# gavrissh/training-operator

Measured on AMD Instinct MI355X. Metric: job×node fit evals/sec + gang placements/sec, 1M-node inventory, 1/2/4/8 GPUs, higher is better.
Workload: dtype int64

## Files before the change

training-operator_amd/csrc/pe_ctx.h:

```cpp
#pragma once

#include <hip/hip_runtime.h>
#include <rccl/rccl.h>

#include <immintrin.h>
#include <pthread.h>
#include <sched.h>

#include <algorithm>
#include <atomic>
#include <cstdlib>
#include <cstring>
#include <exception>
#include <functional>
#include <memory>
#include <mutex>
#include <new>
#include <stdexcept>
#include <string>
#include <thread>
#include <vector>

#include "pe_hostx.h"
#include "pe_kernels.h"
#include "pe_ledger_plan.h"
#include "pe_resolver.h"
#include "pe_slice_plan.h"
#include "placement.h"

namespace pe_engine {

using pe::ReqRec;

template <class T>
struct DevBuf {
  T* p = nullptr;
  size_t n = 0;
  hipError_t ensure(size_t count, unsigned flags = 0) {
    if (count <= n && p) return hipSuccess;
    if (p) (void)hipFree(p);
    p = nullptr;
    n = 0;
    const size_t bytes = std::max<size_t>(count, 1) * sizeof(T);
    hipError_t e = hipErrorOutOfMemory;
    if (flags) {
      e = hipExtMallocWithFlags((void**)&p, bytes, flags);
      if (e != hipSuccess) (void)hipGetLastError();
    }
    if (e != hipSuccess) e = hipMalloc((void**)&p, bytes);
    if (e == hipSuccess) n = count;
    return e;
  }
  void release() {
    if (p) (void)hipFree(p);
    p = nullptr;
    n = 0;
  }
};

template <class T>
struct HostBuf {
  T* p = nullptr;
  T* dev = nullptr;
  size_t n = 0;
  hipError_t ensure(size_t count, unsigned flags = hipHostMallocDefault) {
    if (count <= n && p) return hipSuccess;
    if (p) (void)hipHostFree(p);
    p = dev = nullptr;
    n = 0;
    hipError_t e = hipHostMalloc((void**)&p, std::max<size_t>(count, 1) * sizeof(T), flags);
    if (e == hipSuccess) std::memset((void*)p, 0, std::max<size_t>(count, 1) * sizeof(T));
    if (e == hipSuccess) e = hipHostGetDevicePointer((void**)&dev, p, 0);
    if (e == hipSuccess) n = count;
    return e;
  }
  void release() {
    if (p) (void)hipHostFree(p);
    p = dev = nullptr;
    n = 0;
  }
};
constexpr unsigned kZeroCopy = hipHostMallocCoherent | hipHostMallocMapped;

class SpinWorker {
 public:
  explicit SpinWorker(int device) : th_([this, device] {
    (void)hipSetDevice(device);
    loop();
  }) {}
  ~SpinWorker() {
    while (state_.load(std::memory_order_acquire) == 1) _mm_pause();
    state_.store(3, std::memory_order_release);
    th_.join();
  }
  void pin(const cpu_set_t& set) { (void)pthread_setaffinity_np(th_.native_handle(), sizeof(set), &set); }
  void post(std::function<void()> f) {
    task_ = std::move(f);
    err_ = nullptr;
    posted_ = true;
    state_.store(1, std::memory_order_release);
  }
  bool busy() const { return state_.load(std::memory_order_acquire) == 1; }
  bool failed() const { return state_.load(std::memory_order_acquire) == 2 && err_ != nullptr; }
  void wait() {
    if (!posted_) return;
    posted_ = false;
    for (int spin = 0; state_.load(std::memory_order_acquire) != 2; ++spin)
      if (spin < 4096) _mm_pause();
      else std::this_thread::yield();
    state_.store(0, std::memory_order_relaxed);
    if (err_) std::rethrow_exception(err_);
  }

 private:
  void loop() {
    int idle = 0;
    for (;;) {
      const int st = state_.load(std::memory_order_acquire);
      if (st == 3) return;
      if (st != 1) {
        if (++idle < 4096) _mm_pause();
        else std::this_thread::yield();
        continue;
      }
      idle = 0;
      try {
        task_();
      } catch (...) {
        err_ = std::current_exception();
      }
      state_.store(2, std::memory_order_release);
    }
  }
  std::atomic<int> state_{0};
  bool posted_ = false;
  std::function<void()> task_;
  std::exception_ptr err_;
  std::thread th_;
};

class SpinQueue {
 public:
  static constexpr unsigned kCap = 8;
  explicit SpinQueue(int device) : th_([this, device] {
    (void)hipSetDevice(device);
    loop();
  }) {}
  ~SpinQueue() {
    while (busy()) _mm_pause();
    stop_.store(true, std::memory_order_release);
    th_.join();
  }
  void pin(const cpu_set_t& set) { (void)pthread_setaffinity_np(th_.native_handle(), sizeof(set), &set); }
  void post(std::function<void()> f) {
    const unsigned t = tail_.load(std::memory_order_relaxed);
    while (t - head_.load(std::memory_order_acquire) >= kCap) _mm_pause();
    q_[t % kCap] = std::move(f);
    tail_.store(t + 1, std::memory_order_release);
  }
  bool busy() const { return head_.load(std::memory_order_acquire) != tail_.load(std::memory_order_acquire); }
  bool failed() const { return failed_.load(std::memory_order_acquire); }
  void wait() {
    for (int spin = 0; busy(); ++spin)
      if (spin < 4096) _mm_pause();
      else std::this_thread::yield();
    if (failed_.load(std::memory_order_acquire)) {
      failed_.store(false, std::memory_order_relaxed);
      std::exception_ptr e = err_;
      err_ = nullptr;
      if (e) std::rethrow_exception(e);
    }
  }

 private:
  void loop() {
    int idle = 0;
    for (;;) {
      const unsigned h = head_.load(std::memory_order_relaxed);
      if (h == tail_.load(std::memory_order_acquire)) {
        if (stop_.load(std::memory_order_acquire)) return;
        if (++idle < 4096) _mm_pause();
        else std::this_thread::yield();
        continue;
      }
      idle = 0;
      if (!failed_.load(std::memory_order_relaxed)) {
        try {
          q_[h % kCap]();
        } catch (...) {
          err_ = std::current_exception();
          failed_.store(true, std::memory_order_release);
        }
      }
      q_[h % kCap] = nullptr;
      head_.store(h + 1, std::memory_order_release);
    }
  }
  std::function<void()> q_[kCap];
  std::atomic<unsigned> head_{0}, tail_{0};
  std::atomic<bool> failed_{false}, stop_{false};
  std::exception_ptr err_;
  std::thread th_;
};


struct PeError {
  int code;
  std::string msg;
};

[[noreturn]] inline void raise(int code, const std::string& msg) { throw PeError{code, msg}; }

inline void hipchk(hipError_t e, const char* what) {
  if (e != hipSuccess) raise(PE_EHIP, std::string(what) + ": " + hipGetErrorString(e));
}

inline void ncclchk(ncclResult_t r, const char* what) {
  if (r != ncclSuccess) raise(PE_ERCCL, std::string(what) + ": " + ncclGetErrorString(r));
}

inline double rccl_timeout_s() {
  const char* e = std::getenv("PE_RCCL_TIMEOUT_S");
  const double s = e ? std::atof(e) : 60.0;
  return s > 0 ? s : 60.0;
}

inline int64_t round_up(int64_t x, int64_t m) { return (x + m - 1) / m * m; }

constexpr int kMaxMergers = 7;
constexpr int PATH_I64 = 1, PATH_I32 = 2, PATH_CODED = 4, PATH_NO_THERM = 8, PATH_PLANES = 16, PATH_PLANES_BLOCKS = 32,
              PATH_LDS = 64;
constexpr int PATHS_ALL = PATH_I64 | PATH_I32 | PATH_CODED | PATH_PLANES | PATH_LDS;

struct AggSeg {
  int64_t j0;
  int32_t nj, ng, nc;
  int64_t bytes;
// ... 111 lines not shown
  pe::SlicePlan sl_plan;
  HostBuf<uint8_t> dm_hin;
  DevBuf<uint8_t> dm_in;
  DevBuf<uint8_t> dm_out;
  HostBuf<uint8_t> dm_hout;
  DevBuf<int32_t> dm_log;
  DevBuf<int32_t> dm_dom;
  DevBuf<int64_t> dm_seg;
  DevBuf<uint32_t> dm_segw;
  HostBuf<int32_t> dm_hoff;
  hipEvent_t dm_ev = nullptr;
  HostBuf<uint8_t> dm_hlarge;
  DevBuf<uint8_t> dm_large;
  DevBuf<int64_t> dm_scratch;
  DevBuf<int32_t> pp_place;
  DevBuf<uint64_t> ff_state;
  HostBuf<uint32_t> ff_hopen;
  pe::LedgerPlan ld_plan;
  HostBuf<pe::LedgerRec> ld_hin;
  DevBuf<pe::LedgerRec> ld_in;
  DevBuf<ReqRec> g_groups;
  DevBuf<uint64_t> g_cand, g_bound;
  DevBuf<int32_t> g_cnt;
  DevBuf<uint8_t> g_out, g_gath;
  DevBuf<int64_t> g_upd;
  DevBuf<uint64_t> g_kn;
  DevBuf<uint32_t> g_lo;
  HostBuf<ReqRec> h_groups, h_groups2;
  HostBuf<ReqRec> h_groupsx[2];
  HostBuf<uint8_t> h_outx[2];
  HostBuf<int64_t> h_updx[2];
  uint32_t walk_gen = 0;
  int pin_cpu = -2;
  HostBuf<uint8_t> h_out, h_out2, h_own;
  HostBuf<uint8_t> h_merged;
  HostBuf<uint8_t> h_xg[4];
  std::vector<const uint64_t*> x_lists;
  std::vector<int32_t> x_ns, x_hd;
  HostBuf<int64_t> h_upd;
  bool walk = true;
  int64_t resort_nodes = 20480;
  int64_t w_est = 0;
  struct WalkSet {
    DevBuf<uint64_t> sk, rmin;
    DevBuf<int64_t> sr, rmax;
    DevBuf<uint32_t> sl, pos, ror, inovl, ovidx, ovlab;
    DevBuf<int64_t> ovres;
    DevBuf<uint64_t> ovkn;
    DevBuf<int32_t> ovl, ovln;
    void release() {
      sk.release(); rmin.release(); sr.release(); rmax.release(); sl.release(); pos.release(); ror.release();
      inovl.release(); ovidx.release(); ovlab.release(); ovres.release(); ovkn.release(); ovl.release(); ovln.release();
    }
  } ws[2];
  int w_cur = 0;
  bool w_pending = false;
  int64_t w_pend_est = 0;
  int64_t w_pend_windows = 0;
  hipStream_t w_s2 = nullptr;
  hipEvent_t w_ev_snap = nullptr, w_ev_done = nullptr;
  DevBuf<uint64_t> w_kin;
  DevBuf<uint32_t> w_slow;
  DevBuf<uint8_t> w_temp;
  DevBuf<uint32_t> w_flush;
  DevBuf<unsigned long long> w_stat;
  DevBuf<uint64_t> g_xstatus;
  pe_stats stats{};

  ~pe_ctx() {
    (void)hipSetDevice(device);
    if (comm_abort.joinable()) comm_abort.join();
    if (stream) (void)hipStreamSynchronize(stream);
    res0.release(); res.release(); labels.release(); island.release(); n_upd.release();
    fit_jobs.release(); fit_jobs32.release(); res32.release(); mask.release();
    code_vals.release(); code_needs.release(); code_jobs.release(); code_x.release(); counts.release(); h_counts.release();
    planes.release(); plane_jobs.release();
    lds_spec_d.release(); lds_vals.release(); lds_codes.release(); lds_ranks.release(); lds_aux.release(); lds_slots.release(); lds_rows.release();
    a_stage.release(); a_outh.release(); a_segoff.release(); a_flag.release(); a_ctr.release();
    for (hipEvent_t e : a_ev) (void)hipEventDestroy(e);
    if (a_h2d) (void)hipStreamSynchronize(a_h2d);
    for (hipEvent_t e : a_ev_h2d) (void)hipEventDestroy(e);
    if (a_h2d) (void)hipStreamDestroy(a_h2d);
    a_dstage.release();
    a_jgo.release(); a_mm.release(); a_rep.release(); a_gco.release(); a_mem.release();
    a_req.release(); a_out.release(); a_fl.release(); a_pres.release(); a_ovf.release();
    aw_stage.release(); aw_outh.release(); aw_dev.release();
    cp_hshapes.release(); cp_hout.release(); cp_shapes.release(); cp_part.release(); cp_out.release();
    lv_leaf.release(); lv_upper.release(); lv_hslots.release(); lv_hnodes.release();
    lv_hin.release(); lv_in.release(); lv_out.release(); lv_hout.release(); lv_split.release(); lv_hsplit.release();
    dm_hin.release(); dm_in.release(); dm_out.release(); dm_hout.release(); dm_log.release(); dm_dom.release();
    dm_seg.release(); dm_segw.release(); dm_hoff.release(); dm_hlarge.release(); dm_large.release(); dm_scratch.release();
    pp_place.release(); ff_state.release(); ff_hopen.release();
    ld_hin.release(); ld_in.release();
    if (dm_ev) (void)hipEventDestroy(dm_ev);
    for (hipEvent_t e : cp_ev)
      if (e) (void)hipEventDestroy(e);
    g_groups.release(); g_cand.release(); g_bound.release(); g_cnt.release(); g_out.release(); g_gath.release();
    g_upd.release(); g_kn.release(); g_lo.release(); h_groups.release(); h_groups2.release(); h_out.release(); h_out2.release(); h_own.release(); h_merged.release(); h_upd.release();
    for (auto& x : h_xg) x.release();
    for (int i = 0; i < 2; ++i) {
      h_groupsx[i].release();
      h_outx[i].release();
      h_updx[i].release();
    }
    if (w_s2) (void)hipStreamSynchronize(w_s2);
    for (auto& x : ws) x.release();
    w_kin.release(); w_slow.release(); w_temp.release(); w_stat.release(); w_flush.release(); g_xstatus.release();
    if (w_ev_snap) (void)hipEventDestroy(w_ev_snap);
    if (w_ev_done) (void)hipEventDestroy(w_ev_done);
    if (w_s2) (void)hipStreamDestroy(w_s2);
    if (comm) (void)ncclCommDestroy(comm);
    if (stream) (void)hipStreamDestroy(stream);
  }
};

namespace pe_engine {

inline void rccl_abort(pe_ctx* ctx) {
  if (!ctx->comm) return;
  ncclComm_t c = ctx->comm;
  ctx->comm = nullptr;
  ctx->comm_aborted = true;
  const int dev = ctx->device;
  ctx->comm_abort = std::thread([c, dev] {
    (void)hipSetDevice(dev);
    (void)ncclCommAbort(c);
  });
}

template <class F>
int guarded(pe_ctx* ctx, F&& body) {
  if (!ctx) return PE_EINVAL;
  std::lock_guard<std::mutex> lk(ctx->mu);
  ctx->err.clear();
  try {
    hipchk(hipSetDevice(ctx->device), "hipSetDevice");
    return body();
  } catch (const PeError& e) {
    ctx->err = e.msg;
    return e.code;
// ... 96 lines not shown
```

training-operator_amd/csrc/pe_engine_greedy.cpp:

```cpp
#include <chrono>
#include <cstdio>
#include <deque>
#include <utility>

#include "pe_ctx.h"
#include "pe_greedy_mode.h"
#include "pe_merge.h"

namespace {

using Clock = std::chrono::steady_clock;
double ms(Clock::duration d) { return std::chrono::duration<double, std::milli>(d).count(); }
double us(Clock::duration d) { return std::chrono::duration<double, std::micro>(d).count(); }
double ms_since(Clock::time_point t) { return ms(Clock::now() - t); }
double us_since(Clock::time_point t) { return us(Clock::now() - t); }

const pe::GreedyLimits kLimits{pe::WK_ROUND,   pe::MG_CAP,  pe::MG_THREADS,        pe::RM_MAX_WORLD,
                               pe::RM_MAX_LDS, kMaxMergers, &pe::cand_group_bytes, &pe::merge_ranked_lds};

uint32_t next_gen(pe_ctx* ctx) {
  if (++ctx->walk_gen == 0) ++ctx->walk_gen;
  return ctx->walk_gen;
}

// ... 107 lines not shown
  hipchk(pe::launch_walk_switch(s, ctx->res.p, ctx->stride, ctx->labels.p, ctx->Ns, ctx->w_slow.p, walk_index(ctx, nx)),
         "launch walk_switch");
  ctx->w_cur = nx;
  ctx->w_pending = false;
  ctx->w_est = ctx->w_pend_est;
  ctx->stats.resorts += 1;
}

template <class At>
bool read_rank_lists(int W, int K, At group_at, const uint64_t** lists, int32_t* ns, uint64_t* L) {
  bool bad = false;
  *L = pe::NO_KEY;
  for (int r = 0; r < W; ++r) {
    const uint8_t* g = group_at(r);
    pe::CandHdr h;
    std::memcpy(&h, g, sizeof(h));
    *L = std::min(*L, h.limit);
    lists[r] = reinterpret_cast<const uint64_t*>(g + sizeof(h));
    bad |= h.n < 0 || h.n > K;
    ns[r] = std::max(0, std::min(h.n, K));
  }
  return !bad;
}

struct GreedyBatch {
  int64_t n_jobs, G;
  const int32_t *job_group_off, *priority, *group_count;
  const int64_t* group_req;
  const uint32_t* group_need;
};

struct Pin {
  cpu_set_t old_set, l3;
  bool on = false;
  Pin(bool no_pin, int rank, int world, int& picked) {
    if (no_pin || pthread_getaffinity_np(pthread_self(), sizeof(old_set), &old_set) != 0) return;
    if (world > 1 && picked == -2) picked = pe::l3_pick(old_set, rank);
    const int cpu = world > 1 ? picked : sched_getcpu();
    if (!pe::l3_cpus(cpu, &l3)) return;
    CPU_AND(&l3, &l3, &old_set);
    on = CPU_COUNT(&l3) >= 3 && pthread_setaffinity_np(pthread_self(), sizeof(l3), &l3) == 0;
  }
  ~Pin() {
    if (on) (void)pthread_setaffinity_np(pthread_self(), sizeof(old_set), &old_set);
  }
};

struct StreamIdle {
  hipStream_t s;
  const SpinQueue* x = nullptr;
  static bool stream_busy(hipStream_t s) {
    const hipError_t e = hipStreamQuery(s);
    if (e == hipErrorNotReady) return true;
    hipchk(e, "walk window stream");
    return false;
  }
  static bool busy(void* u) {
    auto* t = static_cast<StreamIdle*>(u);
    if (t->x && t->x->failed()) const_cast<SpinQueue*>(t->x)->wait();
    return (t->x && t->x->busy()) || stream_busy(t->s);
  }
};

struct DumpClose {
  FILE*& f;
  ~DumpClose() {
    if (f) std::fclose(f);
  }
};

struct TraceOut {
  int& helper_cpu;
  const bool& on;
  std::vector<double>& a; std::vector<double>& b; std::vector<double>& c;
  std::vector<double>& d; std::vector<double>& e; std::vector<double>& f;
  ~TraceOut() {
    if (!on || a.empty()) return;
    auto pr = [](const char* n, std::vector<double>& v) {
      if (v.empty()) return;
      std::sort(v.begin(), v.end());
      double sum = 0;
      for (double x : v) sum += x;
      std::fprintf(stderr, "%s n %zu sum %.2f ms mean %.1f us p10 %.1f p50 %.1f p90 %.1f max %.1f\n", n, v.size(),
                   sum / 1e3, sum / v.size(), v[v.size() / 10], v[v.size() / 2], v[v.size() * 9 / 10], v.back());
    };
    pr("wait   ", a);
    pr("resolve", b);
    pr("post   ", c);
    pr("xspin  ", d);
    pr("xmerge ", e);
    pr("xblock ", f);
    auto sib = [](int cpu) {
      char path[128], buf[64] = {0};
      std::snprintf(path, sizeof path, "/sys/devices/system/cpu/cpu%d/topology/thread_siblings_list", cpu);
      FILE* f = std::fopen(path, "r");
      if (f) {
        if (!std::fgets(buf, sizeof buf, f)) buf[0] = 0;
        std::fclose(f);
      }
      buf[std::strcspn(buf, "\n")] = 0;
      return std::string(buf);
    };
    const int mc = sched_getcpu();
    std::fprintf(stderr, "cpus: main %d (siblings %s) helper %d (siblings %s)\n", mc, sib(mc).c_str(), helper_cpu,
                 helper_cpu >= 0 ? sib(helper_cpu).c_str() : "-");
  }
};

struct EventsFree {
  std::vector<std::pair<hipEvent_t, hipEvent_t>>& v;
  ~EventsFree() {
    for (auto& p : v) {
      (void)hipEventDestroy(p.first);
      (void)hipEventDestroy(p.second);
    }
  }
};

struct XWait {
  std::unique_ptr<SpinQueue>& w;
  ~XWait() {
    if (w) try {
        w->wait();
      } catch (...) {
      }
  }
};

struct Flight {
  std::vector<int32_t> groups;
  pe::Cursor end;
  int buf = 0;
  size_t ver = 0;
};

struct GreedyRun {
  pe_ctx* const ctx;
  const pe::GreedyKnobs kn;
  const pe::GreedyMode m;
  pe::Resolver& R;
  const uint32_t* const group_need;
  pe_host_exchange* const hx;
  const hipStream_t s;
  const size_t gb;
  const int Wmax, nwaves;
  int k_win;
  const bool async_resort, wev, wflush;
  const int64_t kResortEarly, kResortLate;
  decltype(&pe::launch_merge_shards) const merge_fn;
  HostBuf<uint8_t>* const h_blob[4];
  HostBuf<ReqRec>* const h_req[4];
  uint8_t* outbuf(int b) const { return h_blob[b]->p; }
  uint8_t* outbufdev(int b) const { return h_blob[b]->dev; }
  HostBuf<ReqRec>& hgroups(int b) const { return *h_req[m.signalled ? b : 0]; }

  FILE* dump = nullptr;
  DumpClose dump_close{dump};
  int64_t dump_left;
  std::vector<double> tr_wait, tr_res, tr_post, tr_xspin, tr_xmerge, tr_xblock;
  int helper_cpu = -1;
  TraceOut trace_out{helper_cpu, kn.trace, tr_wait, tr_res, tr_post, tr_xspin, tr_xmerge, tr_xblock};
  std::vector<std::pair<hipEvent_t, hipEvent_t>> walk_events;
  EventsFree events_free{walk_events};
  int64_t walk_launch_groups = 0;
  std::vector<pe::GroupCands> cands;
  int cb = 0;
  std::unique_ptr<SpinWorker> worker;
  const Pin& pin;
  const uint8_t* last_blob = nullptr;
  uint32_t buf_gen[4] = {0, 0, 0, 0};
  int buf_k[4];
  pe::WindowFeed feed;
  StreamIdle stream_idle;
  const double coll_tmo;
  double feed_spin_seen = 0;
  std::unique_ptr<SpinQueue> xworker;
  std::vector<std::unique_ptr<SpinWorker>> xmergers;
  XWait xwait_exit{xworker};
  std::deque<Flight> fl;
  std::vector<std::vector<pe::Update>> hist;
  size_t n_app = 0;
  int next_buf = 0, upd_slot = 0;
  bool posted = false;
  std::vector<pe::Update> seed, upd;
  std::vector<std::pair<const std::vector<pe::Update>*, int>> to_apply;
  std::vector<Flight*> to_scan;
  Clock::time_point t_setup, t_loop;

  GreedyRun(pe_ctx* c, const GreedyBatch& batch, const pe::GreedyKnobs& knobs, const pe::GreedyMode& mode,
            pe::Resolver& resolver, const Pin& pinned)
      : ctx(c), kn(knobs), m(mode), R(resolver), group_need(batch.group_need),
        hx(pe::hx_is(c->exchange) ? static_cast<pe_host_exchange*>(c->exchange_user) : nullptr), s(c->stream),
        gb(pe::cand_group_bytes(mode.K)), Wmax(c->window_groups),
        nwaves((int)std::max<int64_t>(1, (c->Ns + pe::SC_SPAN - 1) / pe::SC_SPAN)), k_win(mode.K0),
        async_resort(mode.walk && knobs.async_resort), wev(mode.walk && knobs.walk_events),
        wflush(mode.walk && knobs.walk_flush), kResortEarly(std::min<int64_t>(4096, c->resort_nodes / 4)),
        kResortLate(std::max<int64_t>(1, c->resort_nodes / 2)),
        merge_fn(mode.ranked ? &pe::launch_merge_ranked : &pe::launch_merge_shards),
        h_blob{&c->h_out, &c->h_out2, &c->h_outx[0], &c->h_outx[1]},
        h_req{&c->h_groups, &c->h_groups2, &c->h_groupsx[0], &c->h_groupsx[1]}, dump_left(knobs.dump_max),
        pin(pinned), buf_k{mode.K, mode.K, mode.K, mode.K}, stream_idle{c->stream},
        coll_tmo(!mode.use_exchange && c->comm ? rccl_timeout_s() : 0.0) {
    open_dump(batch);
    if (m.pipelined) {
      worker.reset(new SpinWorker(ctx->device));
      if (pin.on) worker->pin(pin.l3);
    }
    if (pin.on) R.pin_helper(pin.l3);
    feed.idle = &StreamIdle::busy;
    feed.idle_user = &stream_idle;
    feed.timeout_s = coll_tmo;
    feed.on_timeout = [](void* u) { rccl_abort(static_cast<pe_ctx*>(u)); };
    feed.timeout_user = ctx;
    if (m.split_x) {
      xworker.reset(new SpinQueue(ctx->device));
      if (pin.on) xworker->pin(pin.l3);
      stream_idle.x = xworker.get();
      if (m.zc_host) {
        for (int t = 1; t < m.T; ++t) {
          xmergers.emplace_back(new SpinWorker(ctx->device));
          if (pin.on) xmergers.back()->pin(pin.l3);
          xmergers.back()->post(&pe::merge_warm);
        }
        xworker->post(&pe::merge_warm);
      }
    }
  }

  void open_dump(const GreedyBatch& b) {
    if (!kn.dump_path) return;
    dump = std::fopen(kn.dump_path, "wb");
    if (!dump) return;
    const int64_t hdr[3] = {b.n_jobs, b.G, (int64_t)m.K};
    std::fwrite(hdr, 8, 3, dump);
    std::fwrite(b.job_group_off, 4, (size_t)b.n_jobs + 1, dump);
    std::fwrite(b.priority, 4, (size_t)b.n_jobs, dump);
    std::fwrite(b.group_count, 4, (size_t)b.G, dump);
    std::fwrite(b.group_req, 8, (size_t)b.G * pe::D, dump);
    std::fwrite(b.group_need, 4, (size_t)b.G, dump);
    std::fwrite(&ctx->n_total, 8, 1, dump);
    std::fwrite(ctx->m_nodes.data(), sizeof(pe::NodeState), ctx->m_nodes.size(), dump);
  }

  void sync_stream(const char* what) {
    if (coll_tmo <= 0) return hipchk(hipStreamSynchronize(s), what);
    const auto ts = Clock::now();
    for (unsigned spin = 1;; ++spin) {
      const hipError_t e = hipStreamQuery(s);
      if (e != hipErrorNotReady) return hipchk(e, what);
      if (spin > 64) std::this_thread::sleep_for(std::chrono::microseconds(20));
      if ((spin & 63) == 0 && std::chrono::duration<double>(Clock::now() - ts).count() > coll_tmo) {
        rccl_abort(ctx);
        throw pe::CollectiveTimeout(std::string(what) + ": the stream did not drain within " +
// ... 118 lines not shown
    for (int t = 1; t < T; ++t) {
      Times* x = &tt[t];
      xmergers[(size_t)t - 1]->wait();
      xmergers[(size_t)t - 1]->post([&timed_share, t, x] { timed_share(t, x); });
    }
    std::exception_ptr err;
    try {
      timed_share(0, &tt[0]);
    } catch (...) {
      err = std::current_exception();
    }
    for (int t = 1; t < T; ++t) try {
        xmergers[(size_t)t - 1]->wait();
      } catch (...) {
        if (!err) err = std::current_exception();
      }
    if (err) std::rethrow_exception(err);
    double busy = 0, spun = 0, merged = 0;
    for (int t = 0; t < T; ++t) {
      busy = std::max(busy, tt[t].busy);
      spun += tt[t].spun;
      merged += tt[t].merged;
    }
    if (trace) {
      tr_xspin.push_back(spun);
      tr_xmerge.push_back(merged);
    }
    const double all_ms = ms_since(t0);
    ctx->stats.xchg_merge_ms += busy;
    ctx->stats.xchg_wait_ms += std::max(0.0, all_ms - busy);
    pe::hx_zc_consumed(hx, *hw);
  }

  void exchange_window(int b, int Wg, uint32_t gen, bool own_direct, const SpinWorker* launcher,
                       const pe::HxWindow* hw = nullptr) {
    if (m.zc_host) return exchange_window_zc(b, Wg, gen, hw);
    const int K = m.K;
    const size_t bytes = (size_t)Wg * gb;
    if (own_direct && ctx->Ns > 0) {
      struct Idle {
        const SpinWorker* l;
        hipStream_t s;
        static bool busy(void* u) {
          auto* x = static_cast<Idle*>(u);
          return (x->l && x->l->busy()) || StreamIdle::stream_busy(x->s);
        }
      } idle{launcher, s};
      pe::WindowFeed own;
      std::vector<pe::GroupCands> own_cands;
      own.idle = &Idle::busy;
      own.idle_user = &idle;
      own.reset(ctx->h_own.p, Wg, K, gen, &own_cands);
      own.wait((size_t)Wg - 1);
    } else {
      hipchk(hipMemcpyAsync(ctx->h_own.p, ctx->g_out.p, bytes, hipMemcpyDeviceToHost, s), "D2H cands");
      hipchk(hipStreamSynchronize(s), "sync own cands");
    }
    const auto tx = Clock::now();
    if (ctx->exchange(ctx->exchange_user, ctx->h_own.p, m.dev_merge ? ctx->h_xg[b].p : outbuf(b), bytes) != 0)
      raise(PE_ERCCL, "exchange callback failed");
    ctx->stats.xchg_wait_ms += ms_since(tx);
    if (m.xhost_merge) {
      const auto tm = Clock::now();
      for (int w = 0; w < Wg; ++w) host_merge_group(ctx->h_xg[b].p, Wg, w, outbuf(b), gen);
      ctx->stats.xchg_merge_ms += ms_since(tm);
    } else if (m.dev_merge) {
      hipchk(merge_fn(s, ctx->h_xg[b].dev, ctx->world, Wg, K, outbufdev(b), gen, 0, nullptr, true),
             "launch merge_shards");
    }
  }

  void launch_lists(const HostBuf<ReqRec>& hg, int b, int Wg, int Kw, uint8_t* dst, uint32_t gen, const pe::HxWindow& hw) {
    const int K = m.K;
    if (m.walk) {
// ... 206 lines not shown
  }

  void restart() {
    fl.clear();
    hist.clear();
    n_app = 0;
    next_buf = 0;
    Flight* f = add_flight(R.cursor());
    if (!f) return;
    if (m.split_x && m.zc_host) {
      const uint32_t gen = next_gen(ctx);
      const pe::HxWindow hw = pe::hx_zc_next(hx);
      enqueue_window(f->groups, f->buf, gen, true, &hw);
      const int b = f->buf, wg = (int)f->groups.size();
      xworker->post([this, b, wg, gen, hw] { exchange_window(b, wg, gen, true, worker.get(), &hw); });
    } else {
      enqueue_window(f->groups, f->buf);
    }
  }

  void plan_post() {
    to_apply.clear();
    to_scan.clear();
    for (; n_app < hist.size(); ++n_app) {
      to_apply.emplace_back(&hist[n_app], upd_slot);
      upd_slot = (upd_slot + 1) % m.upd_slots;
    }
    while ((int)fl.size() < m.depth + 1)
      if (Flight* f = add_flight(fl.back().end)) to_scan.push_back(f);
      else break;
  }

  void post_scan() {
    worker->post([this, to_apply = to_apply, to_scan = to_scan] {
      const auto tp = Clock::now();
      if (kn.trace) helper_cpu = sched_getcpu();
      for (const auto& a : to_apply) enqueue_apply(*a.first, a.second);
      for (Flight* f : to_scan) enqueue_window(f->groups, f->buf);
      if (kn.trace) tr_post.push_back(us_since(tp));
    });
  }

  void post_split() {
    plan_post();
    struct XWin {
      int buf, wg;
      uint32_t gen;
      pe::HxWindow hw;
    };
    std::vector<XWin> xs;
    std::vector<std::pair<Flight*, XWin>> ws;
    for (Flight* f : to_scan) {
      const uint32_t gen = next_gen(ctx);
      xs.push_back(XWin{f->buf, (int)f->groups.size(), gen, m.zc_host ? pe::hx_zc_next(hx) : pe::HxWindow{}});
      ws.emplace_back(f, xs.back());
    }
    const auto txb = Clock::now();
    if (!m.zc_host) xworker->wait();
    if (kn.trace) tr_xblock.push_back(us_since(txb));
    worker->post([this, to_apply = to_apply, ws] {
      const auto tp = Clock::now();
      if (kn.trace) helper_cpu = sched_getcpu();
      for (const auto& a : to_apply) enqueue_apply(*a.first, a.second);
      for (const auto& w : ws)
        enqueue_window(w.first->groups, w.first->buf, w.second.gen, true, m.zc_host ? &w.second.hw : nullptr);
      if (kn.trace) tr_post.push_back(us_since(tp));
    });
// ... 35 lines not shown
        try {
          worker->wait();
        } catch (...) {
        }
        if (xworker) xworker->wait();
        throw;
      }
      worker->wait();
      const bool landed = consumed && R.cursor() == cur.end && fl.size() > 1;
      if (landed && !R.done()) {
        hist.push_back(std::move(upd));
        upd = {};
        fl.pop_front();
        if (m.early_post) {
          plan_post();
          post_scan();
          posted = true;
        }
        continue;
      }
      if (xworker) xworker->wait();
      sync_stream("sync speculative");
      for (; n_app < hist.size(); ++n_app) {
        enqueue_apply(hist[n_app], 0);
        sync_stream("sync apply");
      }
      enqueue_apply(upd, 0);
      if (R.done()) break;
      if (!consumed) k_win = m.K;
      restart();
    }
    t_loop = Clock::now();
    if (xworker) xworker->wait();
    sync_stream("sync greedy");
    walk_drop_pending(ctx);
  }

  void walk_stats() {
    if (!m.walk) return;
    unsigned long long wc[2] = {0, 0};
    hipchk(hipMemcpy(wc, ctx->w_stat.p, sizeof(wc), hipMemcpyDeviceToHost), "D2H walk counters");
    ctx->stats.walk_rounds += (int64_t)wc[0];
    ctx->stats.walk_overlay += (int64_t)wc[1];
    ctx->stats.walk_groups += walk_launch_groups;
    ctx->stats.walk_prepass += walk_launch_groups * ((ctx->Ns + pe::WK_ROUND - 1) / pe::WK_ROUND);
    for (auto& p : walk_events) {
      float t = 0.f;
      hipchk(hipEventElapsedTime(&t, p.first, p.second), "event elapsed");
      ctx->stats.walk_ms += t;
    }
  }
};

int64_t check_batch(GreedyBatch& b, const int32_t* out_pod_node, const int32_t* out_job_status) {
  need_ptr(b.job_group_off, "job_group_off");
  need_ptr(b.priority, "priority");
  need_ptr(out_job_status, "out_job_status");
  check_offsets(b.job_group_off, b.n_jobs, -1, "job_group_off");
  b.G = b.job_group_off[b.n_jobs];
  int64_t P = 0;
  if (b.G > 0) {
    need_ptr(b.group_count, "group_count");
    need_ptr(b.group_req, "group_req");
    check_req(b.group_req, b.G, "group_req");
    for (int64_t g = 0; g < b.G; ++g) {
      if (b.group_count[g] < 0) raise(PE_EINVAL, "negative group_count");
      P += b.group_count[g];
    }
  }
  if (P > 0) need_ptr(out_pod_node, "out_pod_node");
  return P;
}

void prep_device(pe_ctx* ctx) {
  hipchk(ctx->g_kn.ensure((size_t)std::max<int64_t>(ctx->stride, 1)), "alloc node keys");
  hipchk(ctx->g_lo.ensure((size_t)2 * std::max<int64_t>(ctx->stride, 1)), "alloc node lows");
  hipchk(pe::launch_prep_nodes(ctx->stream, ctx->res.p, ctx->stride, ctx->Ns, (uint64_t)ctx->begin, ctx->g_kn.p,
                               ctx->g_lo.p),
         "launch prep_nodes");
  hipchk(ctx->w_stat.ensure(2), "alloc walk counters");
  hipchk(hipMemsetAsync(ctx->w_stat.p, 0, 2 * sizeof(unsigned long long), ctx->stream), "memset walk counters");
  if (ctx->walk && ctx->Ns > 0) walk_resort(ctx);
}

pe::GreedyFacts greedy_facts(const pe_ctx* ctx) {
  pe::GreedyFacts f;
  f.world = ctx->world;
  f.rank = ctx->rank;
  f.has_comm = ctx->comm != nullptr;
  f.has_exchange = ctx->exchange != nullptr;
  f.hx = pe::hx_is(ctx->exchange);
  f.hx_slot_bytes = f.hx ? pe::hx_slot_bytes(static_cast<const pe_host_exchange*>(ctx->exchange_user)) : 0;
  f.ctx_walk = ctx->walk;
  f.has_nodes = ctx->Ns > 0;
  f.pipeline = ctx->pipeline;
  f.topk = ctx->topk;
  f.window_groups = ctx->window_groups;
  return f;
}

bool zc_agreed(pe_ctx* ctx, int K) {
  pe_host_exchange* const hx = static_cast<pe_host_exchange*>(ctx->exchange_user);
  if (ctx->zc_hx != hx) {
    const uint8_t ok = ctx->world <= pe::HX_ZC_MAX_WORLD && pe::hx_zc_register(hx) &&
                               (size_t)ctx->window_groups * pe::cand_group_bytes(K) <= pe::hx_slot_bytes(hx) ? 1 : 0;
    std::vector<uint8_t> all((size_t)ctx->world, 0);
    if (ctx->exchange(ctx->exchange_user, &ok, all.data(), 1) != 0) raise(PE_ERCCL, "exchange callback failed");
    ctx->zc_ok = std::all_of(all.begin(), all.end(), [](uint8_t v) { return v == 1; });
    ctx->zc_hx = hx;
  }
  return ctx->zc_ok;
}

// ... 28 lines not shown
      hipchk(ctx->h_xg[b].ensure((size_t)Wmax * gb * ctx->world, kZeroCopy), "alloc pinned gathered");
}

}

extern "C" {

int pe_place_greedy(pe_ctx* ctx, int64_t n_jobs, const int32_t* job_group_off, const int32_t* priority,
                    const int32_t* group_count, const int64_t* group_req, const uint32_t* group_need,
                    int32_t* out_pod_node, int32_t* out_job_status) {
  return guarded(ctx, [&]() -> int {
    const auto t0 = Clock::now();
    if (!ctx->loaded) raise(PE_ESTATE, "no inventory loaded");
    if (ctx->comm_aborted)
      raise(PE_ERCCL, "the RCCL communicator was aborted after a window's all-gather timed out; recreate the context");
    if (n_jobs < 0) raise(PE_EINVAL, "n_jobs < 0");
    if (n_jobs == 0) return PE_OK;
    GreedyBatch batch{n_jobs, 0, job_group_off, priority, group_count, group_req, group_need};
    const int64_t P = check_batch(batch, out_pod_node, out_job_status);
    std::vector<uint32_t> no_need;
    if (!batch.group_need) {
      no_need.assign((size_t)std::max<int64_t>(batch.G, 1), 0u);
      batch.group_need = group_need = no_need.data();
    }
    prep_device(ctx);
    const auto t_prep = Clock::now();
    if (ctx->resolver) ctx->resolver->reset(n_jobs, job_group_off, priority, group_count, group_req, group_need);
    else ctx->resolver.reset(new pe::Resolver(n_jobs, job_group_off, priority, group_count, group_req, group_need));
    pe::Resolver& R = *ctx->resolver;
    R.set_mirror(pe::Mirror{ctx->m_nodes.data(), ctx->n_total});
    const auto t_res = Clock::now();

    const pe::GreedyKnobs kn = pe::GreedyKnobs::from_env();
    const Pin pin(kn.no_pin, ctx->rank, ctx->world, ctx->pin_cpu);
    const pe::GreedyFacts facts = greedy_facts(ctx);
    const bool zc = pe::greedy_zc_wanted(facts, kn, kLimits) && zc_agreed(ctx, pe::greedy_mode_base(facts, kn, kLimits).K);
    const pe::GreedyMode m = pe::greedy_mode(facts, kn, kLimits, zc);
    size_buffers(ctx, kn, m);

    GreedyRun run(ctx, batch, kn, m, R, pin);
    run.run();
    run.walk_stats();
    if (P > 0) std::memcpy(out_pod_node, R.pod_node().data(), (size_t)P * 4);
    std::memcpy(out_job_status, R.job_status().data(), (size_t)n_jobs * 4);
    ctx->stats.rescans += R.rescans();
    ctx->stats.pods_placed += R.pods_placed();
    ctx->stats.jobs_placed += R.jobs_placed();
    ctx->stats.jobs_failed += R.jobs_failed();
    ctx->stats.last_greedy_ms = ms_since(t0);
    if (kn.trace)
      std::fprintf(stderr, "greedy phases (us): checks+prep %.0f resolver %.0f setup %.0f loop %.0f tail %.0f\n",
                   us(t_prep - t0), us(t_res - t_prep), us(run.t_setup - t_res), us(run.t_loop - run.t_setup),
                   us_since(run.t_loop));
    return PE_OK;
  });
}

}
```

training-operator_amd/csrc/pe_resolver.cpp:

```cpp
#include "pe_resolver.h"

#include <algorithm>
#include <chrono>
#include <stdexcept>
#include <string>
#include <cstring>
#include <numeric>
#include <utility>
#include <cstdio>
#include <cstdlib>

#include <immintrin.h>
#include <pthread.h>
#include <sched.h>
#ifdef PE_RES_PROF
#include <x86intrin.h>
#endif

namespace pe {
#ifdef PE_RES_PROF
struct ResProf { long cgroups = 0, cskip = 0, cdirty = 0; unsigned long long p1 = 0, p2 = 0, p3 = 0, la = 0, ka = 0, st = 0, seed = 0, keys = 0, skip = 0, place = 0, fin = 0, other = 0; long skips = 0, pods = 0, groups = 0, dirty = 0, scored = 0, sready = 0, slocal = 0, sfull = 0;
  ~ResProf() { std::fprintf(stderr, "keys split: lookahead %.1fM keys_all %.1fM seed top %.1fM | place split: choose+fetch %.1fM m %.1fM upsert..key %.1fM\n", la / 1e6, ka / 1e6, st / 1e6, p1 / 1e6, p2 / 1e6, p3 / 1e6); std::fprintf(stderr, "cycles seed %.1fM keys %.1fM skip %.1fM place %.1fM fin %.1fM | skips %ld pods %ld | per group: dirty %.0f scored %.1f\n", seed / 1e6, keys / 1e6, skip / 1e6, place / 1e6, fin / 1e6, skips, pods, (double)dirty / groups, (double)scored / groups); std::fprintf(stderr, "seed tops: helper %ld local %ld full %ld\n", sready, slocal, sfull); std::fprintf(stderr, "window conflicts: %ld of %ld groups depend on an earlier group of their window (%ld via a skipped list entry, %ld via a chosen changed node)\n", cgroups, groups, cskip, cdirty); } };
static ResProf rp;
#define RP_T() __rdtsc()
// ... 480 lines not shown
    while (h < gc.size() && seeds.contains((int64_t)(gc.keys[h] & 0xFFFFFFull))) ++h;
  top.head = h;
  seeds.keys_all(q, need, gc.limit, out, idx);
  int n = 0;
  bool trunc = false;
  for (int32_t i : idx) {
    const uint64_t k = out[(size_t)i];
    if (k >= gc.limit) continue;
    if (n == SeedTop::kTop) {
      trunc = true;
      if (k >= top.key[n - 1]) continue;
      --n;
    }
    int j = n++;
    for (; j > 0 && top.key[j - 1] > k; --j) top.key[j] = top.key[j - 1];
    top.key[j] = k;
  }
  top.n = n;
  top.truncated = trunc;
}

SeedScorer::~SeedScorer() {
  if (!th_) return;
  stop();
  state_.store(3, std::memory_order_seq_cst);
  {
    std::lock_guard<std::mutex> lk(park_mu_);
    park_cv_.notify_one();
  }
  th_->join();
}

void SeedScorer::pin(const cpu_set_t& set) {
  pin_set_ = set;
  have_pin_ = true;
  if (th_) (void)pthread_setaffinity_np(th_->native_handle(), sizeof(set), &set);
}

void SeedScorer::start(const DirtySet* seeds, const std::vector<int32_t>* groups,
                       const std::vector<GroupCands>* cands, const int64_t* scan_req, const uint32_t* need,
                       const WindowFeed* feed, const NodeState* mirror, int64_t mirror_n) {
  seeds_ = seeds;
  mirror_ = mirror;
  mirror_n_ = mirror ? mirror_n : 0;
  groups_ = groups;
  cands_ = cands;
  feed_ = feed;
  req_ = scan_req;
  need_ = need;
  if (cap_ < groups->size()) {
    cap_ = std::max<size_t>(groups->size(), 2 * cap_);
    slots_.reset(new TopSlot[cap_]);
    gen_ = 0;
  }
  if (++gen_ == 0) {
    for (size_t i = 0; i < cap_; ++i) slots_[i].gen.store(0, std::memory_order_relaxed);
    gen_ = 1;
  }
  main_wi_.store(0, std::memory_order_relaxed);
  if (!th_) {
    th_.reset(new std::thread([this] { loop(); }));
#ifndef PE_SEED_TEST_YIELD
    cpu_set_t set;
    if (have_pin_) (void)pthread_setaffinity_np(th_->native_handle(), sizeof(pin_set_), &pin_set_);
    else if (l3_cpus(sched_getcpu(), &set)) (void)pthread_setaffinity_np(th_->native_handle(), sizeof(set), &set);
#endif
// ... 547 lines not shown
```

Before: 46470 billion.

## Persist parked helper threads across greedy calls and cache CPU pinning

Replaces the per-call SpinWorker and SpinQueue helper threads with persistent ParkedWorker and ParkedQueue objects stored in the context. Between calls they sleep on a condition variable and are woken by a lease when a run starts. The L3 affinity set is cached, and pthread_setaffinity is skipped when it would not change anything. The walk-counter readback becomes an async copy into pinned memory before the final sync, replacing a separate blocking hipMemcpy. This removes thread creation, join and redundant syscalls on every greedy call, at the cost of wake latency and more lifecycle complexity.

```diff
diff --git a/training-operator_amd/csrc/pe_ctx.h b/training-operator_amd/csrc/pe_ctx.h
--- a/training-operator_amd/csrc/pe_ctx.h
+++ b/training-operator_amd/csrc/pe_ctx.h
@@ -24,6 +24,7 @@
 #include "pe_hostx.h"
 #include "pe_kernels.h"
 #include "pe_ledger_plan.h"
+#include "pe_parked_worker.h"
 #include "pe_resolver.h"
 #include "pe_slice_plan.h"
 #include "placement.h"
@@ -82,127 +83,9 @@
 };
 constexpr unsigned kZeroCopy = hipHostMallocCoherent | hipHostMallocMapped;
 
-class SpinWorker {
- public:
-  explicit SpinWorker(int device) : th_([this, device] {
-    (void)hipSetDevice(device);
-    loop();
-  }) {}
-  ~SpinWorker() {
-    while (state_.load(std::memory_order_acquire) == 1) _mm_pause();
-    state_.store(3, std::memory_order_release);
-    th_.join();
-  }
-  void pin(const cpu_set_t& set) { (void)pthread_setaffinity_np(th_.native_handle(), sizeof(set), &set); }
-  void post(std::function<void()> f) {
-    task_ = std::move(f);
-    err_ = nullptr;
-    posted_ = true;
-    state_.store(1, std::memory_order_release);
-  }
-  bool busy() const { return state_.load(std::memory_order_acquire) == 1; }
-  bool failed() const { return state_.load(std::memory_order_acquire) == 2 && err_ != nullptr; }
-  void wait() {
-    if (!posted_) return;
-    posted_ = false;
-    for (int spin = 0; state_.load(std::memory_order_acquire) != 2; ++spin)
-      if (spin < 4096) _mm_pause();
-      else std::this_thread::yield();
-    state_.store(0, std::memory_order_relaxed);
-    if (err_) std::rethrow_exception(err_);
-  }
-
- private:
-  void loop() {
-    int idle = 0;
-    for (;;) {
-      const int st = state_.load(std::memory_order_acquire);
-      if (st == 3) return;
-      if (st != 1) {
-        if (++idle < 4096) _mm_pause();
-        else std::this_thread::yield();
-        continue;
-      }
-      idle = 0;
-      try {
-        task_();
-      } catch (...) {
-        err_ = std::current_exception();
-      }
-      state_.store(2, std::memory_order_release);
-    }
-  }
-  std::atomic<int> state_{0};
-  bool posted_ = false;
-  std::function<void()> task_;
-  std::exception_ptr err_;
-  std::thread th_;
-};
-
-class SpinQueue {
- public:
-  static constexpr unsigned kCap = 8;
-  explicit SpinQueue(int device) : th_([this, device] {
-    (void)hipSetDevice(device);
-    loop();
-  }) {}
-  ~SpinQueue() {
-    while (busy()) _mm_pause();
-    stop_.store(true, std::memory_order_release);
-    th_.join();
-  }
-  void pin(const cpu_set_t& set) { (void)pthread_setaffinity_np(th_.native_handle(), sizeof(set), &set); }
-  void post(std::function<void()> f) {
-    const unsigned t = tail_.load(std::memory_order_relaxed);
-    while (t - head_.load(std::memory_order_acquire) >= kCap) _mm_pause();
-    q_[t % kCap] = std::move(f);
-    tail_.store(t + 1, std::memory_order_release);
-  }
-  bool busy() const { return head_.load(std::memory_order_acquire) != tail_.load(std::memory_order_acquire); }
-  bool failed() const { return failed_.load(std::memory_order_acquire); }
-  void wait() {
-    for (int spin = 0; busy(); ++spin)
-      if (spin < 4096) _mm_pause();
-      else std::this_thread::yield();
-    if (failed_.load(std::memory_order_acquire)) {
-      failed_.store(false, std::memory_order_relaxed);
-      std::exception_ptr e = err_;
-      err_ = nullptr;
-      if (e) std::rethrow_exception(e);
-    }
-  }
-
- private:
-  void loop() {
-    int idle = 0;
-    for (;;) {
-      const unsigned h = head_.load(std::memory_order_relaxed);
-      if (h == tail_.load(std::memory_order_acquire)) {
-        if (stop_.load(std::memory_order_acquire)) return;
-        if (++idle < 4096) _mm_pause();
-        else std::this_thread::yield();
-        continue;
-      }
-      idle = 0;
-      if (!failed_.load(std::memory_order_relaxed)) {
-        try {
-          q_[h % kCap]();
-        } catch (...) {
-          err_ = std::current_exception();
-          failed_.store(true, std::memory_order_release);
-        }
-      }
-      q_[h % kCap] = nullptr;
-      head_.store(h + 1, std::memory_order_release);
-    }
-  }
-  std::function<void()> q_[kCap];
-  std::atomic<unsigned> head_{0}, tail_{0};
-  std::atomic<bool> failed_{false}, stop_{false};
-  std::exception_ptr err_;
-  std::thread th_;
-};
-
+inline std::function<void()> helper_init(int device) {
+  return [device] { (void)hipSetDevice(device); };
+}
 
 struct PeError {
   int code;
@@ -380,6 +263,11 @@
   HostBuf<int64_t> h_updx[2];
   uint32_t walk_gen = 0;
   int pin_cpu = -2;
+  cpu_set_t pin_l3;
+  int pin_l3_cpu = -1;
+  std::unique_ptr<pe::ParkedWorker> g_worker;
+  std::unique_ptr<pe::ParkedQueue> g_xworker;
+  std::vector<std::unique_ptr<pe::ParkedWorker>> g_xmergers;
   HostBuf<uint8_t> h_out, h_out2, h_own;
   HostBuf<uint8_t> h_merged;
   HostBuf<uint8_t> h_xg[4];
@@ -412,12 +300,16 @@
   DevBuf<uint8_t> w_temp;
   DevBuf<uint32_t> w_flush;
   DevBuf<unsigned long long> w_stat;
+  HostBuf<unsigned long long> h_wstat;
   DevBuf<uint64_t> g_xstatus;
   pe_stats stats{};
 
   ~pe_ctx() {
     (void)hipSetDevice(device);
     if (comm_abort.joinable()) comm_abort.join();
+    g_xmergers.clear();
+    g_xworker.reset();
+    g_worker.reset();
     if (stream) (void)hipStreamSynchronize(stream);
     res0.release(); res.release(); labels.release(); island.release(); n_upd.release();
     fit_jobs.release(); fit_jobs32.release(); res32.release(); mask.release();
@@ -453,7 +345,7 @@
     }
     if (w_s2) (void)hipStreamSynchronize(w_s2);
     for (auto& x : ws) x.release();
-    w_kin.release(); w_slow.release(); w_temp.release(); w_stat.release(); w_flush.release(); g_xstatus.release();
+    w_kin.release(); w_slow.release(); w_temp.release(); w_stat.release(); h_wstat.release(); w_flush.release(); g_xstatus.release();
     if (w_ev_snap) (void)hipEventDestroy(w_ev_snap);
     if (w_ev_done) (void)hipEventDestroy(w_ev_done);
     if (w_s2) (void)hipStreamDestroy(w_s2);
diff --git a/training-operator_amd/csrc/pe_engine_greedy.cpp b/training-operator_amd/csrc/pe_engine_greedy.cpp
--- a/training-operator_amd/csrc/pe_engine_greedy.cpp
+++ b/training-operator_amd/csrc/pe_engine_greedy.cpp
@@ -163,23 +163,31 @@
 
 struct Pin {
   cpu_set_t old_set, l3;
-  bool on = false;
-  Pin(bool no_pin, int rank, int world, int& picked) {
+  bool on = false, moved = false;
+  Pin(bool no_pin, pe_ctx* ctx) {
     if (no_pin || pthread_getaffinity_np(pthread_self(), sizeof(old_set), &old_set) != 0) return;
-    if (world > 1 && picked == -2) picked = pe::l3_pick(old_set, rank);
-    const int cpu = world > 1 ? picked : sched_getcpu();
-    if (!pe::l3_cpus(cpu, &l3)) return;
-    CPU_AND(&l3, &l3, &old_set);
-    on = CPU_COUNT(&l3) >= 3 && pthread_setaffinity_np(pthread_self(), sizeof(l3), &l3) == 0;
+    if (ctx->world > 1 && ctx->pin_cpu == -2) ctx->pin_cpu = pe::l3_pick(old_set, ctx->rank);
+    const int cpu = ctx->world > 1 ? ctx->pin_cpu : sched_getcpu();
+    if (cpu < 0 || cpu >= CPU_SETSIZE) return;
+    if (ctx->pin_l3_cpu < 0 || !CPU_ISSET(cpu, &ctx->pin_l3)) {
+      ctx->pin_l3_cpu = -1;
+      if (!pe::l3_cpus(cpu, &ctx->pin_l3)) return;
+      ctx->pin_l3_cpu = cpu;
+    }
+    CPU_AND(&l3, &ctx->pin_l3, &old_set);
+    if (CPU_COUNT(&l3) < 3) return;
+    moved = !CPU_EQUAL(&l3, &old_set);
+    on = !moved || pthread_setaffinity_np(pthread_self(), sizeof(l3), &l3) == 0;
+    moved = moved && on;
   }
   ~Pin() {
-    if (on) (void)pthread_setaffinity_np(pthread_self(), sizeof(old_set), &old_set);
+    if (moved) (void)pthread_setaffinity_np(pthread_self(), sizeof(old_set), &old_set);
   }
 };
 
 struct StreamIdle {
   hipStream_t s;
-  const SpinQueue* x = nullptr;
+  const pe::ParkedQueue* x = nullptr;
   static bool stream_busy(hipStream_t s) {
     const hipError_t e = hipStreamQuery(s);
     if (e == hipErrorNotReady) return true;
@@ -188,7 +196,7 @@
   }
   static bool busy(void* u) {
     auto* t = static_cast<StreamIdle*>(u);
-    if (t->x && t->x->failed()) const_cast<SpinQueue*>(t->x)->wait();
+    if (t->x && t->x->failed()) const_cast<pe::ParkedQueue*>(t->x)->wait();
     return (t->x && t->x->busy()) || stream_busy(t->s);
   }
 };
@@ -248,15 +256,34 @@
   }
 };
 
-struct XWait {
-  std::unique_ptr<SpinQueue>& w;
-  ~XWait() {
-    if (w) try {
-        w->wait();
-      } catch (...) {
-      }
+template <class T>
+struct Lease {
+  T* t = nullptr;
+  Lease() = default;
+  Lease(const Lease&) = delete;
+  Lease& operator=(const Lease&) = delete;
+  void take(T* x) {
+    t = x;
+    t->wake();
+  }
+  T* operator->() const { return t; }
+  T* get() const { return t; }
+  explicit operator bool() const { return t != nullptr; }
+  void drain() const {
+    if (t) t->drain();
+  }
+  ~Lease() {
+    if (!t) return;
+    t->drain();
+    t->park();
   }
 };
+
+template <class T>
+T* helper_of(std::unique_ptr<T>& slot, int device) {
+  if (!slot) slot.reset(new T(helper_init(device)));
+  return slot.get();
+}
 
 struct Flight {
   std::vector<int32_t> groups;
@@ -296,7 +323,7 @@
   int64_t walk_launch_groups = 0;
   std::vector<pe::GroupCands> cands;
   int cb = 0;
-  std::unique_ptr<SpinWorker> worker;
+  Lease<pe::ParkedWorker> worker;
   const Pin& pin;
   const uint8_t* last_blob = nullptr;
   uint32_t buf_gen[4] = {0, 0, 0, 0};
@@ -305,9 +332,8 @@
   StreamIdle stream_idle;
   const double coll_tmo;
   double feed_spin_seen = 0;
-  std::unique_ptr<SpinQueue> xworker;
-  std::vector<std::unique_ptr<SpinWorker>> xmergers;
-  XWait xwait_exit{xworker};
+  Lease<pe::ParkedQueue> xworker;
+  std::deque<Lease<pe::ParkedWorker>> xmergers;
   std::deque<Flight> fl;
   std::vector<std::vector<pe::Update>> hist;
   size_t n_app = 0;
@@ -317,6 +343,14 @@
   std::vector<std::pair<const std::vector<pe::Update>*, int>> to_apply;
   std::vector<Flight*> to_scan;
   Clock::time_point t_setup, t_loop;
+  struct TasksOver {
+    GreedyRun* r;
+    ~TasksOver() {
+      r->worker.drain();
+      r->xworker.drain();
+      for (auto& x : r->xmergers) x.drain();
+    }
+  } tasks_over{this};
 
   GreedyRun(pe_ctx* c, const GreedyBatch& batch, const pe::GreedyKnobs& knobs, const pe::GreedyMode& mode,
             pe::Resolver& resolver, const Pin& pinned)
@@ -334,7 +368,7 @@
         coll_tmo(!mode.use_exchange && c->comm ? rccl_timeout_s() : 0.0) {
     open_dump(batch);
     if (m.pipelined) {
-      worker.reset(new SpinWorker(ctx->device));
+      worker.take(helper_of(ctx->g_worker, ctx->device));
       if (pin.on) worker->pin(pin.l3);
     }
     if (pin.on) R.pin_helper(pin.l3);
@@ -344,12 +378,14 @@
     feed.on_timeout = [](void* u) { rccl_abort(static_cast<pe_ctx*>(u)); };
     feed.timeout_user = ctx;
     if (m.split_x) {
-      xworker.reset(new SpinQueue(ctx->device));
+      xworker.take(helper_of(ctx->g_xworker, ctx->device));
       if (pin.on) xworker->pin(pin.l3);
       stream_idle.x = xworker.get();
       if (m.zc_host) {
+        if ((int)ctx->g_xmergers.size() < m.T - 1) ctx->g_xmergers.resize((size_t)m.T - 1);
         for (int t = 1; t < m.T; ++t) {
-          xmergers.emplace_back(new SpinWorker(ctx->device));
+          xmergers.emplace_back();
+          xmergers.back().take(helper_of(ctx->g_xmergers[(size_t)t - 1], ctx->device));
           if (pin.on) xmergers.back()->pin(pin.l3);
           xmergers.back()->post(&pe::merge_warm);
         }
@@ -534,14 +570,14 @@
     pe::hx_zc_consumed(hx, *hw);
   }
 
-  void exchange_window(int b, int Wg, uint32_t gen, bool own_direct, const SpinWorker* launcher,
+  void exchange_window(int b, int Wg, uint32_t gen, bool own_direct, const pe::ParkedWorker* launcher,
                        const pe::HxWindow* hw = nullptr) {
     if (m.zc_host) return exchange_window_zc(b, Wg, gen, hw);
     const int K = m.K;
     const size_t bytes = (size_t)Wg * gb;
     if (own_direct && ctx->Ns > 0) {
       struct Idle {
-        const SpinWorker* l;
+        const pe::ParkedWorker* l;
         hipStream_t s;
         static bool busy(void* u) {
           auto* x = static_cast<Idle*>(u);
@@ -814,7 +850,7 @@
   }
 
   void post_scan() {
-    worker->post([this, to_apply = to_apply, to_scan = to_scan] {
+    worker->post([this] {
       const auto tp = Clock::now();
       if (kn.trace) helper_cpu = sched_getcpu();
       for (const auto& a : to_apply) enqueue_apply(*a.first, a.second);
@@ -916,14 +952,16 @@
     }
     t_loop = Clock::now();
     if (xworker) xworker->wait();
+    if (m.walk)
+      hipchk(hipMemcpyAsync(ctx->h_wstat.p, ctx->w_stat.p, 2 * sizeof(unsigned long long), hipMemcpyDeviceToHost, s),
+             "D2H walk counters");
     sync_stream("sync greedy");
     walk_drop_pending(ctx);
   }
 
   void walk_stats() {
     if (!m.walk) return;
-    unsigned long long wc[2] = {0, 0};
-    hipchk(hipMemcpy(wc, ctx->w_stat.p, sizeof(wc), hipMemcpyDeviceToHost), "D2H walk counters");
+    const unsigned long long* wc = ctx->h_wstat.p;
     ctx->stats.walk_rounds += (int64_t)wc[0];
     ctx->stats.walk_overlay += (int64_t)wc[1];
     ctx->stats.walk_groups += walk_launch_groups;
@@ -963,6 +1001,7 @@
                                ctx->g_lo.p),
          "launch prep_nodes");
   hipchk(ctx->w_stat.ensure(2), "alloc walk counters");
+  hipchk(ctx->h_wstat.ensure(2), "alloc pinned walk counters");
   hipchk(hipMemsetAsync(ctx->w_stat.p, 0, 2 * sizeof(unsigned long long), ctx->stream), "memset walk counters");
   if (ctx->walk && ctx->Ns > 0) walk_resort(ctx);
 }
@@ -1057,7 +1096,7 @@
     const auto t_res = Clock::now();
 
     const pe::GreedyKnobs kn = pe::GreedyKnobs::from_env();
-    const Pin pin(kn.no_pin, ctx->rank, ctx->world, ctx->pin_cpu);
+    const Pin pin(kn.no_pin, ctx);
     const pe::GreedyFacts facts = greedy_facts(ctx);
     const bool zc = pe::greedy_zc_wanted(facts, kn, kLimits) && zc_agreed(ctx, pe::greedy_mode_base(facts, kn, kLimits).K);
     const pe::GreedyMode m = pe::greedy_mode(facts, kn, kLimits, zc);
diff --git a/training-operator_amd/csrc/pe_parked_worker.h b/training-operator_amd/csrc/pe_parked_worker.h
--- /dev/null
+++ b/training-operator_amd/csrc/pe_parked_worker.h
@@ -0,0 +1,205 @@
+#pragma once
+
+#include <immintrin.h>
+#include <pthread.h>
+#include <sched.h>
+
+#include <atomic>
+#include <condition_variable>
+#include <exception>
+#include <functional>
+#include <mutex>
+#include <thread>
+
+namespace pe {
+
+class ParkedThread {
+ public:
+  void wake() {
+    if (awake_.load(std::memory_order_relaxed)) return;
+    {
+      std::lock_guard<std::mutex> lk(mu_);
+      awake_.store(true, std::memory_order_release);
+    }
+    cv_.notify_one();
+  }
+  void park() { awake_.store(false, std::memory_order_release); }
+  bool parked() const { return !awake_.load(std::memory_order_acquire); }
+  void pin(const cpu_set_t& set) {
+    if (have_pin_ && CPU_EQUAL(&pin_set_, &set)) return;
+    pin_set_ = set;
+    have_pin_ = true;
+    (void)pthread_setaffinity_np(th_.native_handle(), sizeof(set), &set);
+  }
+
+ protected:
+  ParkedThread() = default;
+  ~ParkedThread() = default;
+  template <class Exit>
+  void idle_step(int& idle, Exit exit) {
+    if (!awake_.load(std::memory_order_acquire)) {
+      std::unique_lock<std::mutex> lk(mu_);
+      cv_.wait(lk, [&] { return awake_.load(std::memory_order_relaxed) || exit(); });
+      idle = 0;
+      return;
+    }
+    if (++idle < 4096) _mm_pause();
+    else std::this_thread::yield();
+  }
+  template <class Set>
+  void stop_thread(Set set_exit) {
+    {
+      std::lock_guard<std::mutex> lk(mu_);
+      set_exit();
+    }
+    cv_.notify_one();
+    th_.join();
+  }
+  std::atomic<bool> awake_{false};
+  std::mutex mu_;
+  std::condition_variable cv_;
+  cpu_set_t pin_set_;
+  bool have_pin_ = false;
+  std::thread th_;
+};
+
+class ParkedWorker : public ParkedThread {
+ public:
+  explicit ParkedWorker(std::function<void()> init) {
+    th_ = std::thread([this, init = std::move(init)] {
+      if (init) init();
+      loop();
+    });
+  }
+  ~ParkedWorker() {
+    while (busy()) _mm_pause();
+    stop_thread([this] { state_.store(3, std::memory_order_release); });
+  }
+  void post(std::function<void()> f) {
+    task_ = std::move(f);
+    err_ = nullptr;
+    posted_ = true;
+    state_.store(1, std::memory_order_release);
+    wake();
+  }
+  bool busy() const { return state_.load(std::memory_order_acquire) == 1; }
+  bool failed() const { return state_.load(std::memory_order_acquire) == 2 && err_ != nullptr; }
+  void wait() {
+    if (!posted_) return;
+    posted_ = false;
+    for (int spin = 0; state_.load(std::memory_order_acquire) != 2; ++spin)
+      if (spin < 4096) _mm_pause();
+      else std::this_thread::yield();
+    state_.store(0, std::memory_order_relaxed);
+    std::exception_ptr e = err_;
+    err_ = nullptr;
+    task_ = nullptr;
+    if (e) std::rethrow_exception(e);
+  }
+  void drain() noexcept {
+    for (int spin = 0; busy(); ++spin)
+      if (spin < 4096) _mm_pause();
+      else std::this_thread::yield();
+    state_.store(0, std::memory_order_relaxed);
+    posted_ = false;
+    err_ = nullptr;
+    task_ = nullptr;
+  }
+
+ private:
+  void loop() {
+    int idle = 0;
+    for (;;) {
+      const int st = state_.load(std::memory_order_acquire);
+      if (st == 3) return;
+      if (st != 1) {
+        idle_step(idle, [this] { const int s = state_.load(std::memory_order_relaxed); return s == 1 || s == 3; });
+        continue;
+      }
+      idle = 0;
+      try {
+        task_();
+      } catch (...) {
+        err_ = std::current_exception();
+      }
+      state_.store(2, std::memory_order_release);
+    }
+  }
+  std::atomic<int> state_{0};
+  bool posted_ = false;
+  std::function<void()> task_;
+  std::exception_ptr err_;
+};
+
+class ParkedQueue : public ParkedThread {
+ public:
+  static constexpr unsigned kCap = 8;
+  explicit ParkedQueue(std::function<void()> init) {
+    th_ = std::thread([this, init = std::move(init)] {
+      if (init) init();
+      loop();
+    });
+  }
+  ~ParkedQueue() {
+    while (busy()) _mm_pause();
+    stop_thread([this] { stop_.store(true, std::memory_order_release); });
+  }
+  void post(std::function<void()> f) {
+    const unsigned t = tail_.load(std::memory_order_relaxed);
+    while (t - head_.load(std::memory_order_acquire) >= kCap) _mm_pause();
+    q_[t % kCap] = std::move(f);
+    tail_.store(t + 1, std::memory_order_release);
+    wake();
+  }
+  bool busy() const { return head_.load(std::memory_order_acquire) != tail_.load(std::memory_order_acquire); }
+  bool failed() const { return failed_.load(std::memory_order_acquire); }
+  void wait() {
+    for (int spin = 0; busy(); ++spin)
+      if (spin < 4096) _mm_pause();
+      else std::this_thread::yield();
+    if (failed_.load(std::memory_order_acquire)) {
+      failed_.store(false, std::memory_order_relaxed);
+      std::exception_ptr e = err_;
+      err_ = nullptr;
+      if (e) std::rethrow_exception(e);
+    }
+  }
+  void drain() noexcept {
+    try {
+      wait();
+    } catch (...) {
+    }
+  }
+
+ private:
+  void loop() {
+    int idle = 0;
+    for (;;) {
+      const unsigned h = head_.load(std::memory_order_relaxed);
+      if (h == tail_.load(std::memory_order_acquire)) {
+        if (stop_.load(std::memory_order_acquire)) return;
+        idle_step(idle, [this, h] {
+          return stop_.load(std::memory_order_relaxed) || h != tail_.load(std::memory_order_relaxed);
+        });
+        continue;
+      }
+      idle = 0;
+      if (!failed_.load(std::memory_order_relaxed)) {
+        try {
+          q_[h % kCap]();
+        } catch (...) {
+          err_ = std::current_exception();
+          failed_.store(true, std::memory_order_release);
+        }
+      }
+      q_[h % kCap] = nullptr;
+      head_.store(h + 1, std::memory_order_release);
+    }
+  }
+  std::function<void()> q_[kCap];
+  std::atomic<unsigned> head_{0}, tail_{0};
+  std::atomic<bool> failed_{false}, stop_{false};
+  std::exception_ptr err_;
+};
+
+}
diff --git a/training-operator_amd/csrc/pe_resolver.cpp b/training-operator_amd/csrc/pe_resolver.cpp
--- a/training-operator_amd/csrc/pe_resolver.cpp
+++ b/training-operator_amd/csrc/pe_resolver.cpp
@@ -536,6 +536,7 @@
 }
 
 void SeedScorer::pin(const cpu_set_t& set) {
+  if (have_pin_ && CPU_EQUAL(&pin_set_, &set)) return;
   pin_set_ = set;
   have_pin_ = true;
   if (th_) (void)pthread_setaffinity_np(th_->native_handle(), sizeof(set), &set);
```

Result: no change. 46480 billion (median of 2 runs) (+0.0%).
